# ZhaozhiQIAN/Hybrid-ODE-NeurIPS-2021

Hardware: AMD Instinct MI355X
Metric: patient-trajectories/sec (fwd+adjoint) at dim=12, T=100 (higher is better)
Workload: dtype f32; 1 GPU; dim12 synthetic, 10000 patients/GPU, T=100, dt=0.125, rk4(3/8), fused rhs+step kernel + discrete-adjoint kernel (split expert/learned wave pipelines); patients_total=10000, launch=hipGraph, lanes_per_patient=auto, theta_grad=True, parallelism=dp1, n_ranks=1, stage_tape=True

## Files before the change

hybrid-ode-neurips-2021_amd/csrc/hode_rk_split.hip:

```cpp
#include <hip/hip_runtime.h>
#include <stdlib.h>

#include "../../include/hode.h"
#include "hode_common.hpp"
#include "hode_host.hpp"
#include "hode_roche.hpp"

namespace hode {

#ifndef HODE_SPLIT_EXPERT_FIRST
#define HODE_SPLIT_EXPERT_FIRST 1
#endif
constexpr int kSplitPatients = 48;

struct SplitArgs {
  const float* __restrict__ t;
  const float* __restrict__ y0;
  const float* __restrict__ dosage;
  const float* __restrict__ dose_times;
  const float* __restrict__ theta;
  const float* __restrict__ w1;
  const float* __restrict__ b1;
  float* __restrict__ h;
  float* __restrict__ tape;
  unsigned long long* dbg;
  float* __restrict__ ltape;
  int* __restrict__ status;
  int B, T, K, perturb;
};

struct SpTimes {
  float t0, t1, dt, ts[4];
  HODE_DEV SpTimes(const float* __restrict__ t, int n, int perturb, int method) {
    t0 = t[n];
    t1 = t[n + 1];
    dt = t1 - t0;
    ts[0] = perturb ? nextafter_up(t0) : t0;
    ts[3] = perturb ? nextafter_down(t1) : t1;
    if (method == HODE_METHOD_RK4_38) {
      ts[1] = add_rn(t0, mul_rn(dt, (float)(1.0 / 3.0)));
      ts[2] = add_rn(t0, mul_rn(dt, (float)(2.0 / 3.0)));
    } else {
      ts[1] = add_rn(t0, mul_rn(0.5f, dt));
      ts[2] = ts[1];
    }
  }
};

template <int METHOD>
HODE_DEV float sp_stage_time(float t0, float t1, int perturb, int q) {
  const float dt = t1 - t0;
  const float c = METHOD == HODE_METHOD_RK4_38 ? (q == 1 ? (float)(1.0 / 3.0) : (q == 2 ? (float)(2.0 / 3.0) : 0.f))
                                               : (q == 0 ? 0.f : 0.5f);
  float tq = add_rn(t0, mul_rn(dt, c));
  tq = q == 3 ? t1 : tq;
  if (perturb) {
    if (q == 0) tq = nextafter_up(t0);
    if (q == 3) tq = nextafter_down(t1);
  }
  return tq;
}

constexpr int kSplitMaxT = 8192;
HODE_DEV void sp_stage_grid(float* __restrict__ tg, const float* __restrict__ t, int T) {
// ... 297 lines not shown
      for (int s = 0; s < NS; ++s) e[s] = *reinterpret_cast<const float4*>(&ring[par][s][slot][0]);
      __builtin_amdgcn_sched_barrier(0);
      dose_step(par, t_c, t_d);
#if HODE_SPLIT_EXPERT_FIRST
      typename Ml::Part pe[4];
#pragma unroll
      for (int s = 0; s < NS; ++s) pe[s] = ml.rhs_expert(e[s]);
#endif
#pragma unroll
      for (int s = 0; s < 4; ++s) k[s] = vsplat<Own>(0.f);
#pragma unroll
      for (int s = 0; s < NS; ++s) {
        const Own Yo = sp_stage_state<METHOD>(s, yo, dt, k[0], k[1], k[2]);
#if HODE_SPLIT_EXPERT_FIRST
        k[s] = ml.rhs_rest(pe[s], Ml::stage(e[s], Yo));
#else
        k[s] = ml.rhs(Ml::stage(e[s], Yo));
#endif
      }
      yo = sp_advance<METHOD>(yo, dt, k[0], k[1], k[2], k[3]);
      Ml::store_own(a.h + (size_t)(n + 1) * row + (size_t)p * D, q, yo);
      if constexpr (TAPE && NLT > 0) Ml::template store_tape<NLT>(a.ltape + (size_t)n * lt_step + lt_lane, k + (NS - NLT));
      HODE_FSTAMP(it)
      __syncthreads();
    };
    for (int it = 1; it < a.T; it += 2) {
      m_iter(it, IC<0>{});
      if (it + 1 < a.T) m_iter(it + 1, IC<1>{});
    }
    if (a.status) {
      if (!vfinite(yo) && live) atomicOr(a.status, HODE_STATUS_NONFINITE);
    }
  }
}

struct SplitBwdArgs {
  const float* __restrict__ t;
  const float* __restrict__ dosage;
  const float* __restrict__ dose_times;
  const float* __restrict__ theta;
  const float* __restrict__ w1;
  const float* __restrict__ b1;
  const float* __restrict__ h;
  const float* __restrict__ grad_h;
  float* __restrict__ grad_y0;
  float* __restrict__ part_ml;
  float* __restrict__ part_th;
  const float* __restrict__ tape;
  const float* __restrict__ ltape;
  int B, T, K, perturb;
  unsigned long long* dbg;
};

template <int METHOD, class V, class F>
HODE_DEV void sp_adjoint_step(V& lam, float dt, F&& vjp) {
  constexpr float c13 = (float)(1.0 / 3.0);
  if constexpr (METHOD == HODE_METHOD_EULER) {
    lam += vjp(0, dt * lam);
  } else if constexpr (METHOD == HODE_METHOD_MIDPOINT) {
    const V a1 = vjp(1, dt * lam);
    lam += a1;
    lam += vjp(0, (0.5f * dt) * a1);
  } else {
    const float w1 = dt * 0.125f, w3 = dt * 0.375f;
    const V a3 = vjp(3, w1 * lam);
    V da = dt * a3;
    V g1 = vfma(w1, lam, da);
    V g2 = vfma(w3, lam, -da);
    const V g = vfma(w3, lam, da);
    lam += a3;
    const V a2 = vjp(2, g);
    da = dt * a2;
    g2 += da;
    g1 = vfma(-c13, da, g1);
    lam += a2;
    const V a1 = vjp(1, g2);
    g1 = vfma(c13, dt * a1, g1);
    lam += a1;
    lam += vjp(0, g1);
  }
}

struct F4 {
  f2 a, b;
  HODE_DEV F4& operator+=(const F4& o) { a += o.a; b += o.b; return *this; }
  HODE_DEV F4 operator-() const { return F4{-a, -b}; }
};
HODE_DEV F4 operator*(float s, const F4& v) { return F4{s * v.a, s * v.b}; }
HODE_DEV F4 vfma(float s, const F4& x, const F4& y) { return F4{vfma(s, x.a, y.a), vfma(s, x.b, y.b)}; }

template <int D, bool CW>
struct SplitBwdShared {
  static constexpr int RD = CW ? 3 : 2;
  static constexpr int M = D - 4;
  float yring[RD][4][kSplitPatients][4];
  float cring[RD][4][kSplitPatients + 1][4];
  float dring[RD][kSplitPatients][8];
  float gring[RD][4][kSplitPatients + 1][4];
  float tdring[RD][kSplitPatients][8];
  float uring[CW ? RD : 1][4][CW ? kSplitPatients : 1][CW ? M : 1];
  float red[4][4][M * D + M];
};

template <int D, int METHOD, bool ABLATE, bool HILL2, bool NEED_TH, bool K1, bool TAPE>
HODE_DEV void split_bwd_body(const SplitBwdArgs& a, SplitBwdShared<D, TAPE>& sh) {
  constexpr int NS = sp_stages<METHOD>();
  typedef MlRows<D> Ml;
  typedef typename Ml::Own Own;
  constexpr int M = Ml::M, MR = Ml::MR, DP = Ml::DP, MP = Ml::MP;
  constexpr bool THW = TAPE && NEED_TH;
  constexpr bool CW = TAPE;
  constexpr int RD = SplitBwdShared<D, TAPE>::RD;
  constexpr int EL = CW ? 2 : 1;
  constexpr int CWAVE = THW ? 5 : 4;
  auto& yring = sh.yring; auto& cring = sh.cring; auto& dring = sh.dring; auto& gring = sh.gring;
  auto& tdring = sh.tdring; auto& uring = sh.uring; auto& red = sh.red;
  extern __shared__ float tg[];
  const int tid = threadIdx.x;
  const int wave = tid >> 6, lane = tid & 63;
  const int b0 = blockIdx.x * kSplitPatients;
  const RocheTheta th = load_theta(a.theta, ABLATE);
  const size_t row = (size_t)a.B * D;
  const int T = a.T;
  const int NIT = T + EL - 1;
  sp_stage_grid(tg, a.t, a.T);
#ifdef HODE_SPLIT_STAMPS
#define HODE_SSTAMP(k) if (a.dbg && blockIdx.x == 0 && lane == 0) a.dbg[(size_t)wave * (a.T + 2) + (k)] = __builtin_amdgcn_s_memtime();
#define HODE_PSTAMP(k, ph) { __builtin_amdgcn_sched_barrier(0); if (a.dbg && blockIdx.x == 0 && wave == 3 && lane == 0) a.dbg[(size_t)6 * (a.T + 2) + 64 + (size_t)(k) * 8 + (ph)] = __builtin_amdgcn_s_memtime(); __builtin_amdgcn_sched_barrier(0); }
  if (a.dbg && blockIdx.x < 8 && lane == 0) a.dbg[(size_t)6 * (a.T + 2) + blockIdx.x * 8 + wave] = __builtin_amdgcn_s_getreg(63492);
#else
#define HODE_SSTAMP(k)
#define HODE_PSTAMP(k, ph)
#endif
  auto run = [&](auto&& iter) {
    for (int k = 0; k < NIT; k += RD) {
      iter(k, IC<0>{});
      if (k + 1 < NIT) iter(k + 1, IC<1>{});
      if constexpr (RD == 3) {
        if (k + 2 < NIT) iter(k + 2, IC<2>{});
      }
    }
  };

  if (wave == 0) {
    const int slot = lane < kSplitPatients ? lane : 0;
    const bool mine = lane < kSplitPatients;
    const bool live = mine && b0 + slot < a.B;
    const int p = min(b0 + slot, a.B - 1);
    const float lv = live ? 1.0f : 0.0f;
    DoseSched<K1> ds;
    ds.dosage = a.dosage[p];
    ds.K = a.K;
    ds.taus = a.dose_times + (size_t)p * a.K;
    ds.tau0 = K1 ? ds.taus[0] : 0.f;
    const float ln_ec50 = log_f32(th.ec50);
    const int cslot = mine ? lane : kSplitPatients;
    if (lane < 16 * RD) (&cring[lane >> 4][(lane >> 2) & 3][kSplitPatients][0])[lane & 3] = 0.f;
    const unsigned lane_h = (unsigned)p * D, lane_t = (unsigned)p * 4;
    MlSlice<4, 1> none;
    MlColSlice<4, 1> nonec;
    GradAcc<4, 1> acc;
    acc.zero();
    float own1[1] = {0.f};

    float tp[4][4];
    auto fetch = [&](int m) {
      const float4 v = *reinterpret_cast<const float4*>(a.h + (size_t)m * row + lane_h);
      tp[0][0] = v.x; tp[0][1] = v.y; tp[0][2] = v.z; tp[0][3] = v.w;
      if constexpr (TAPE) {
        const float* __restrict__ tape_m = a.tape + (size_t)m * (NS - 1) * a.B * 4;
#pragma unroll
        for (int s = 1; s < NS; ++s) {
          const float4 u = *reinterpret_cast<const float4*>(tape_m + ((unsigned)(s - 1) * (unsigned)a.B * 4u + lane_t));
          tp[s][0] = u.x; tp[s][1] = u.y; tp[s][2] = u.z; tp[s][3] = u.w;
        }
      }
    };
    auto publish = [&](int m, int par) {
      if constexpr (TAPE) {
        if (mine) {
#pragma unroll
          for (int s = 0; s < NS; ++s)
            *reinterpret_cast<float4*>(&yring[par][s][slot][0]) = make_float4(tp[s][0], tp[s][1], tp[s][2], tp[s][3]);
        }
      } else {
        const SpTimes st(a.t, m, a.perturb, METHOD);
        const f2 ya = pair2(tp[0][0], tp[0][1]), yb = pair2(tp[0][2], tp[0][3]);
        f2 ka[4], kb[4];
#pragma unroll
        for (int s = 0; s < 4; ++s) ka[s] = kb[s] = splat2(0.f);
#pragma unroll
        for (int s = 0; s < NS; ++s) {
          const f2 Ya = sp_stage_state<METHOD>(s, ya, st.dt, ka[0], ka[1], ka[2]);
          const f2 Yb = sp_stage_state<METHOD>(s, yb, st.dt, kb[0], kb[1], kb[2]);
          const DoseVal dv = ds.at(st.ts[s], th.kel);
          if (mine) {
            *reinterpret_cast<float4*>(&yring[par][s][slot][0]) = make_float4(Ya.x, Ya.y, Yb.x, Yb.y);
            dring[par][slot][s] = dv.v;
            dring[par][slot][4 + s] = dv.dk;
          }
          if (s + 1 < NS) {
            const float Y[4] = {Ya.x, Ya.y, Yb.x, Yb.y};
            float k[4];
            roche_rhs<4, 1, ABLATE, HILL2>(th, none, dv.v, Y, k, own1);
            ka[s] = pair2(k[0], k[1]);
            kb[s] = pair2(k[2], k[3]);
          }
        }
      }
    };

    F4 lam;
    {
      const float4 g4 = *reinterpret_cast<const float4*>(a.grad_h + (size_t)(T - 1) * row + (size_t)p * D);
      lam.a = lv * pair2(g4.x, g4.y);
      lam.b = lv * pair2(g4.z, g4.w);
    }
    if (T >= 2) {
      fetch(T - 2);
      publish(T - 2, 0);
    }
    __syncthreads();
    auto e_iter = [&](int k, auto SI) {
      constexpr int S = decltype(SI)::value;
      constexpr int par = (S + 1) % RD;
      if (T - 3 - k >= 0) fetch(T - 3 - k);
      if (k >= EL && k <= T + EL - 2) {
        const int m = T - k + EL - 2;
        const float dt = tg[m + 1] - tg[m];
        float Y[4][4];
        F4 cs[4];
        DoseVal dv[4];
        {
          const float4 d0 = *reinterpret_cast<const float4*>(&dring[par][slot][0]);
          const float4 d1 = *reinterpret_cast<const float4*>(&dring[par][slot][4]);
          dv[0].v = d0.x; dv[1].v = d0.y; dv[2].v = d0.z; dv[3].v = d0.w;
          dv[0].dk = d1.x; dv[1].dk = d1.y; dv[2].dk = d1.z; dv[3].dk = d1.w;
          if constexpr (THW) {
            *reinterpret_cast<float4*>(&tdring[S][slot][0]) = d0;
            *reinterpret_cast<float4*>(&tdring[S][slot][4]) = d1;
          }
        }
#pragma unroll
        for (int s = 0; s < NS; ++s) {
          const float4 yv = *reinterpret_cast<const float4*>(&yring[par][s][slot][0]);
          const float4 cv = *reinterpret_cast<const float4*>(&cring[par][s][cslot][0]);
          Y[s][0] = yv.x; Y[s][1] = yv.y; Y[s][2] = yv.z; Y[s][3] = yv.w;
          cs[s].a = pair2(cv.x, cv.y);
          cs[s].b = pair2(cv.z, cv.w);
        }
        sp_adjoint_step<METHOD>(lam, dt, [&](int s, const F4& gs) {
          const float g[4] = {gs.a.x, gs.a.y, gs.b.x, gs.b.y};
          float av[4];
          if constexpr (THW) {
            if (mine) *reinterpret_cast<float4*>(&gring[S][s][slot][0]) = make_float4(g[0], g[1], g[2], g[3]);
          }
          roche_vjp<4, 1, ABLATE, HILL2, NEED_TH && !THW>(th, none, nonec, ln_ec50, dv[s], Y[s], own1, g, 0, av, acc);
          F4 r = cs[s];
          r.a += pair2(av[0], av[1]);
          r.b += pair2(av[2], av[3]);
          return r;
        });
        const float4 g4 = *reinterpret_cast<const float4*>(a.grad_h + (size_t)m * row + lane_h);
        lam.a = vfma(lv, pair2(g4.x, g4.y), lam.a);
        lam.b = vfma(lv, pair2(g4.z, g4.w), lam.b);
      }
      if (T - 3 - k >= 0) publish(T - 3 - k, par);
      HODE_SSTAMP(k)
      __syncthreads();
    };
    run(e_iter);
    if (live) *reinterpret_cast<float4*>(a.grad_y0 + (size_t)p * D) = make_float4(lam.a.x, lam.a.y, lam.b.x, lam.b.y);
    if constexpr (!THW) {
#pragma unroll
      for (int i = 0; i < kNTheta; ++i) {
        const float v = row_sum(NEED_TH ? acc.dth[i] : 0.f);
        if ((lane & 15) == 0) red[0][lane >> 4][i] = v;
      }
      __builtin_amdgcn_fence(__ATOMIC_SEQ_CST, "wavefront");
      if (lane < kNTheta)
        a.part_th[(size_t)blockIdx.x * kNTheta + lane] = (red[0][0][lane] + red[0][1][lane]) + (red[0][2][lane] + red[0][3][lane]);
    }
  } else if (THW && wave == 4) {
    const int slot = lane < kSplitPatients ? lane : 0;
    const bool mine = lane < kSplitPatients;
    const int p = min(b0 + slot, a.B - 1);
    const int gslot = mine ? lane : kSplitPatients;
    const float ln_ec50 = log_f32(th.ec50);
    if (lane < 16 * RD) (&gring[lane >> 4][(lane >> 2) & 3][kSplitPatients][0])[lane & 3] = 0.f;
    const unsigned lane_h = (unsigned)p * D, lane_t = (unsigned)p * 4;
    float dth[kNTheta];
#pragma unroll
    for (int i = 0; i < kNTheta; ++i) dth[i] = 0.f;
    float tp[4][4];
    auto fetch = [&](int m) {
      const float4 v = *reinterpret_cast<const float4*>(a.h + (size_t)m * row + lane_h);
      tp[0][0] = v.x; tp[0][1] = v.y; tp[0][2] = v.z; tp[0][3] = v.w;
      const float* __restrict__ tape_m = a.tape + (size_t)m * (NS - 1) * a.B * 4;
#pragma unroll
      for (int s = 1; s < NS; ++s) {
        const float4 u = *reinterpret_cast<const float4*>(tape_m + ((unsigned)(s - 1) * (unsigned)a.B * 4u + lane_t));
        tp[s][0] = u.x; tp[s][1] = u.y; tp[s][2] = u.z; tp[s][3] = u.w;
      }
    };
    auto theta_step = [&](int gpar) {
      const float4 d0 = *reinterpret_cast<const float4*>(&tdring[gpar][slot][0]);
      const float4 d1 = *reinterpret_cast<const float4*>(&tdring[gpar][slot][4]);
      const float dvv[4] = {d0.x, d0.y, d0.z, d0.w}, dvk[4] = {d1.x, d1.y, d1.z, d1.w};
#pragma unroll
      for (int si = 0; si < NS; ++si) {
        const int s = NS - 1 - si;
        const float4 gv = *reinterpret_cast<const float4*>(&gring[gpar][s][gslot][0]);
        DoseVal dv;
        dv.v = dvv[s]; dv.dk = dvk[s];
        const float g[4] = {gv.x, gv.y, gv.z, gv.w};
        roche_theta_grad<ABLATE, HILL2>(th, ln_ec50, dv, tp[s], g, dth);
      }
    };
    __syncthreads();
    auto t_iter = [&](int k, auto SI) {
      constexpr int S = decltype(SI)::value;
      constexpr int gpar = (S + RD - 1) % RD;
      if (k >= EL + 1) theta_step(gpar);
      if (k >= EL && T - k + EL - 2 >= 0) fetch(T - k + EL - 2);
      HODE_SSTAMP(k)
      __syncthreads();
    };
    run(t_iter);
    if (T >= 2) theta_step((NIT - 1) % RD);
#pragma unroll
    for (int i = 0; i < kNTheta; ++i) {
      const float v = row_sum(dth[i]);
      if ((lane & 15) == 0) red[0][lane >> 4][i] = v;
    }
    __builtin_amdgcn_fence(__ATOMIC_SEQ_CST, "wavefront");
    if (lane < kNTheta)
      a.part_th[(size_t)blockIdx.x * kNTheta + lane] = (red[0][0][lane] + red[0][1][lane]) + (red[0][2][lane] + red[0][3][lane]);
  } else if (CW && wave == CWAVE) {
    const int slot = lane < kSplitPatients ? lane : 0;
    const bool mine = lane < kSplitPatients;
    float wq[M][4];
#pragma unroll
    for (int j = 0; j < M; ++j)
#pragma unroll
      for (int q = 0; q < 4; ++q) wq[j][q] = a.w1[j * D + q];
    __syncthreads();
    auto c_iter = [&](int k, auto SI) {
      constexpr int S = decltype(SI)::value;
      constexpr int cpar = (S + RD - 1) % RD;
      if (k >= 1 && k - 1 <= T - 2) {
        float u[NS][M];
#pragma unroll
        for (int s = 0; s < NS; ++s) {
#pragma unroll
          for (int j4 = 0; j4 < M; j4 += 4) {
            const float4 v = *reinterpret_cast<const float4*>(&uring[cpar][s][slot][j4]);
            u[s][j4] = v.x; u[s][j4 + 1] = v.y; u[s][j4 + 2] = v.z; u[s][j4 + 3] = v.w;
          }
        }
        __builtin_amdgcn_sched_barrier(0);
#pragma unroll
        for (int s = 0; s < NS; ++s) {
          float c[4];
#pragma unroll
          for (int q = 0; q < 4; ++q) {
            if constexpr (MR == 2) {
              float cq = 0.f;
#pragma unroll
              for (int j = 0; j < M; ++j) cq = __builtin_fmaf(wq[j][q], u[s][j], cq);
              c[q] = cq;
            } else {
              float cx = 0.f, cy = 0.f;
#pragma unroll
              for (int jp = 0; jp < MP; ++jp) {
                cx = __builtin_fmaf(wq[2 * jp][q], u[s][2 * jp], cx);
                cy = __builtin_fmaf(wq[2 * jp + 1][q], u[s][2 * jp + 1], cy);
              }
              c[q] = cx + cy;
            }
          }
          if (mine) *reinterpret_cast<float4*>(&cring[cpar][s][slot][0]) = make_float4(c[0], c[1], c[2], c[3]);
        }
      }
      HODE_SSTAMP(k)
      __syncthreads();
    };
    run(c_iter);
  } else {
    const int q = lane & 3;
    const int slot = (wave - 1) * 16 + (lane >> 2);
    const bool live = b0 + slot < a.B;
    const int p = min(b0 + slot, a.B - 1);
    const float lv = live ? 1.0f : 0.0f;
    Ml ml;
    ml.load(a.w1, a.b1, q);
    typename Ml::Elem wc[Ml::NU];
    f2 wtp[Ml::NU];
    if constexpr (MR == 2) {
#pragma unroll
      for (int j = 0; j < M; ++j) {
        wc[j] = a.w1[j * D + q];
        wtp[j] = pair2(a.w1[j * D + 4 + 2 * q], a.w1[j * D + 4 + 2 * q + 1]);
      }
    } else {
#pragma unroll
      for (int jp = 0; jp < MP; ++jp) {
        wc[jp] = pair2(a.w1[(2 * jp) * D + q], a.w1[(2 * jp + 1) * D + q]);
        wtp[jp] = pair2(a.w1[(2 * jp) * D + 4 + q], a.w1[(2 * jp + 1) * D + 4 + q]);
      }
    }
    f2 dw[Ml::NW];
    Own db = vsplat<Own>(0.f);
#pragma unroll
    for (int i = 0; i < Ml::NW; ++i) dw[i] = splat2(0.f);
    DoseSched<K1> ds;
    ds.dosage = a.dosage[p];
    ds.K = a.K;
    ds.taus = a.dose_times + (size_t)p * a.K;
    ds.tau0 = K1 ? ds.taus[0] : 0.f;
    Own lam = lv * Ml::load_own(a.grad_h + (size_t)(T - 1) * row + (size_t)p * D, q);
    Own yo_nx, gh_nx;
    constexpr int NLT = TAPE ? sp_ltape_stages<METHOD>() : 0;
    const size_t lt_step = (size_t)a.B * 4 * NLT * MR;
    const unsigned lt_lane = ((unsigned)p * 4 + q) * NLT * MR;
    Own lt_nx[NLT > 0 ? NLT : 1], lt_n2[NLT > 0 ? NLT : 1];
    {
      const int m0 = T >= 2 ? T - 2 : 0;
      const int m1 = m0 >= 1 ? m0 - 1 : 0;
      yo_nx = Ml::load_own(a.h + (size_t)m0 * row + (size_t)p * D, q);
      gh_nx = Ml::load_own(a.grad_h + (size_t)m0 * row + (size_t)p * D, q);
      if constexpr (NLT > 0) {
        Ml::template load_tape<NLT>(a.ltape + (size_t)m0 * lt_step + lt_lane, lt_nx);
        Ml::template load_tape<NLT>(a.ltape + (size_t)m1 * lt_step + lt_lane, lt_n2);
      }
    }
    __syncthreads();
    auto m_iter = [&](int k, auto SI) {
      constexpr int par = decltype(SI)::value;
      if (k <= T - 2) {
        HODE_PSTAMP(k, 0)
        const int m = T - 2 - k;
        const float t0 = tg[m], t1 = tg[m + 1];
        const float dt = t1 - t0;
        const Own yo = yo_nx, gh = gh_nx;
        Own lt[NLT > 0 ? NLT : 1];
#pragma unroll
        for (int i = 0; i < NLT; ++i) { lt[i] = lt_nx[i]; lt_nx[i] = lt_n2[i]; }
        {
          const int mn = m >= 1 ? m - 1 : 0;
          yo_nx = Ml::load_own(a.h + (size_t)mn * row + (size_t)p * D, q);
          gh_nx = Ml::load_own(a.grad_h + (size_t)mn * row + (size_t)p * D, q);
          if constexpr (NLT > 0) Ml::template load_tape<NLT>(a.ltape + (size_t)(m >= 2 ? m - 2 : 0) * lt_step + lt_lane, lt_n2);
        }
        typename Ml::Stage Y[4];
        Own so[4];
        float4 e[4];
#pragma unroll
        for (int s = 0; s < NS; ++s) e[s] = *reinterpret_cast<const float4*>(&yring[par][s][slot][0]);
        __builtin_amdgcn_sched_barrier(0);
        HODE_PSTAMP(k, 1)
        if constexpr (TAPE) {
          const DoseVal dq = ds.at(sp_stage_time<METHOD>(t0, t1, a.perturb, q), th.kel);
          dring[par][slot][q] = dq.v;
          if constexpr (NEED_TH) dring[par][slot][4 + q] = dq.dk;
        }
#if HODE_SPLIT_EXPERT_FIRST
        typename Ml::Part pe[4];
#pragma unroll
        for (int s = 0; s < NS - NLT; ++s) pe[s] = ml.rhs_expert(e[s]);
#endif
#pragma unroll
        for (int s = 0; s < 4; ++s) so[s] = vsplat<Own>(0.f);
#pragma unroll
        for (int s = 0; s < NS; ++s) {
          const Own Yo = sp_stage_state<METHOD>(s, yo, dt, so[0], so[1], so[2]);
          Y[s] = Ml::stage(e[s], Yo);
          if (s >= NS - NLT) so[s] = lt[s - (NS - NLT) < 0 ? 0 : s - (NS - NLT)];
#if HODE_SPLIT_EXPERT_FIRST
          else so[s] = ml.rhs_rest(pe[s], Y[s]);
#else
          else so[s] = ml.rhs(Y[s]);
#endif
        }
        HODE_PSTAMP(k, 2)
        sp_adjoint_step<METHOD>(lam, dt, [&](int s, Own gs) {
          HODE_PSTAMP(k, 6 - s)
          const Own u = gs * vfma(-so[s], so[s], vsplat<Own>(1.0f));
          db += u;
          Ml::outer_acc(dw, u, Y[s]);
          if constexpr (CW) {
            if constexpr (MR == 2) *reinterpret_cast<float2*>(&uring[par][s][slot][2 * q]) = make_float2(u.x, u.y);
            else uring[par][s][slot][q] = u;
          }
          typename Ml::Gath uf;
          Ml::gather(u, uf.v);
          if constexpr (MR == 2) {
            float cq = 0.f;
            f2 av = splat2(0.f), av1 = splat2(0.f);
#pragma unroll
            for (int j = 0; j < M; j += 2) {
              if constexpr (!CW) cq = __builtin_fmaf(wc[j], uf.v[j], cq);
              av = vfma(wtp[j], uf.v[j], av);
              if constexpr (!CW) cq = __builtin_fmaf(wc[j + 1], uf.v[j + 1], cq);
              av1 = vfma(wtp[j + 1], uf.v[j + 1], av1);
            }
            if constexpr (!CW) cring[par][s][slot][q] = cq;
            return av + av1;
          } else {
            f2 c2 = splat2(0.f), a2 = splat2(0.f);
#pragma unroll
            for (int jp = 0; jp < MP; ++jp) {
              if constexpr (!CW) c2 = vfma(wc[jp], uf.v[jp], c2);
              a2 = vfma(wtp[jp], uf.v[jp], a2);
            }
            if constexpr (!CW) cring[par][s][slot][q] = hsum(c2);
            return hsum(a2);
          }
        });
        lam = vfma(lv, gh, lam);
        HODE_PSTAMP(k, 7)
      }
      HODE_SSTAMP(k)
      __syncthreads();
    };
    run(m_iter);
    if (live) Ml::store_own(a.grad_y0 + (size_t)p * D, q, lam);
    float* out = a.part_ml + ((size_t)blockIdx.x * 3 + (wave - 1)) * (M * D + M);
    const bool writer = (lane & 15) < 4;
    float* mine = &red[wave][lane >> 4][0];
#pragma unroll
    for (int r = 0; r < MR; ++r) {
#pragma unroll
      for (int i = 0; i < D; ++i) {
        const float v = row_sum_stride4(Ml::dw_at(dw, r, i));
        if (writer) mine[(q * MR + r) * D + i] = v;
      }
      float dbr;
      if constexpr (MR == 2) dbr = r == 0 ? db.x : db.y;
      else dbr = db;
      const float vb = row_sum_stride4(dbr);
      if (writer) mine[M * D + q * MR + r] = vb;
    }
    __builtin_amdgcn_fence(__ATOMIC_SEQ_CST, "wavefront");
    for (int c = lane; c < M * D + M; c += 64)
      out[c] = (red[wave][0][c] + red[wave][1][c]) + (red[wave][2][c] + red[wave][3][c]);
  }
}

__global__ __launch_bounds__(64) void split_fold_kernel(const float* __restrict__ part_ml, const float* __restrict__ part_th,
                                                        int nblk, int P_ml, int n_w, float* __restrict__ gw,
                                                        float* __restrict__ gb, float* __restrict__ gth, int need_th,
                                                        int overwrite) {
  const int j = blockIdx.x;
  const int lane = threadIdx.x;
  const bool ml = j < P_ml;
  const float* src = ml ? part_ml + j : part_th + (j - P_ml);
  const int rows = ml ? 3 * nblk : nblk;
  const int stride = ml ? P_ml : kNTheta;
  float s = 0.f;
  for (int base = 0; base < rows; base += 64 * 8) {
    float v[8];
#pragma unroll
    for (int q = 0; q < 8; ++q) {
      const int w = base + lane + 64 * q;
      v[q] = w < rows ? src[(size_t)w * stride] : 0.f;
    }
#pragma unroll
    for (int q = 0; q < 8; ++q) s += v[q];
  }
  s = wave_sum(s);
  if (lane != 0) return;
  float* dst = nullptr;
  if (ml) dst = j < n_w ? (gw ? gw + j : nullptr) : (gb ? gb + (j - n_w) : nullptr);
  else if (gth) dst = gth + (j - P_ml);
  if (!dst) return;
  if (!ml && !need_th) s = 0.f;
  *dst = overwrite ? s : *dst + s;
}

#ifndef HODE_SPLIT_WPE_FWD
#define HODE_SPLIT_WPE_FWD 2
#endif
#ifndef HODE_SPLIT_WPE_BWD
#define HODE_SPLIT_WPE_BWD 2
#endif
#ifndef HODE_SPLIT_WPE_BWD_MIN
#define HODE_SPLIT_WPE_BWD_MIN 1
#endif

template <int D, int METHOD, bool ABLATE, bool NEED_TH, bool TAPE>
__global__ __launch_bounds__(384) __attribute__((amdgpu_waves_per_eu(HODE_SPLIT_WPE_BWD_MIN, HODE_SPLIT_WPE_BWD))) void split_bwd_kernel(SplitBwdArgs a) {
  __shared__ __attribute__((aligned(16))) SplitBwdShared<D, TAPE> sh;
  const bool hill2 = ABLATE || (a.theta[0] == 2.0f && a.theta[1] == 2.0f);
  if (hill2 && a.K == 1) split_bwd_body<D, METHOD, ABLATE, true, NEED_TH, true, TAPE>(a, sh);
  else if (hill2) split_bwd_body<D, METHOD, ABLATE, true, NEED_TH, false, TAPE>(a, sh);
  else split_bwd_body<D, METHOD, ABLATE, false, NEED_TH, false, TAPE>(a, sh);
}

template <int D, int METHOD, bool ABLATE, bool TAPE>
__global__ __launch_bounds__(256) __attribute__((amdgpu_waves_per_eu(1, HODE_SPLIT_WPE_FWD))) void split_fwd_kernel(SplitArgs a) {
  const bool hill2 = ABLATE || (a.theta[0] == 2.0f && a.theta[1] == 2.0f);
  if (hill2 && a.K == 1) split_fwd_body<D, METHOD, ABLATE, true, true, TAPE>(a);
  else if (hill2) split_fwd_body<D, METHOD, ABLATE, true, false, TAPE>(a);
  else split_fwd_body<D, METHOD, ABLATE, false, false, TAPE>(a);
}

}

namespace {

template <int D, bool ABLATE>
int split_method(const hode_solve_desc* d, const hode::SplitArgs& a, hipStream_t s) {
  const dim3 grid((d->batch + hode::kSplitPatients - 1) / hode::kSplitPatients), block(256);
  const size_t lds = (size_t)(d->n_times + 3) * sizeof(float);
#define HODE_SPLIT_FWD(M)                                                                                 \
  if (a.tape) hipLaunchKernelGGL((hode::split_fwd_kernel<D, M, ABLATE, true>), grid, block, lds, s, a);   \
  else hipLaunchKernelGGL((hode::split_fwd_kernel<D, M, ABLATE, false>), grid, block, lds, s, a);
  switch (d->method) {
    case HODE_METHOD_EULER: HODE_SPLIT_FWD(HODE_METHOD_EULER) break;
    case HODE_METHOD_MIDPOINT: HODE_SPLIT_FWD(HODE_METHOD_MIDPOINT) break;
    default: HODE_SPLIT_FWD(HODE_METHOD_RK4_38) break;
  }
  return hode::hip_fail(hipGetLastError(), "split kernel launch");
}

}

namespace {

template <int D, bool ABLATE>
int split_bwd_method(const hode_solve_desc* d, const hode::SplitBwdArgs& a, hipStream_t s) {
  const dim3 grid((d->batch + hode::kSplitPatients - 1) / hode::kSplitPatients), block(256);
  const size_t lds = (size_t)(d->n_times + 3) * sizeof(float);
#define HODE_SPLIT_BWD(M)                                                                                        \
  if (d->need_theta_grad) {                                                                                      \
    if (a.tape) hipLaunchKernelGGL((hode::split_bwd_kernel<D, M, ABLATE, true, true>), grid, dim3(384), lds, s, a); \
    else hipLaunchKernelGGL((hode::split_bwd_kernel<D, M, ABLATE, true, false>), grid, block, lds, s, a);          \
  } else {                                                                                                       \
    if (a.tape) hipLaunchKernelGGL((hode::split_bwd_kernel<D, M, ABLATE, false, true>), grid, dim3(320), lds, s, a); \
    else hipLaunchKernelGGL((hode::split_bwd_kernel<D, M, ABLATE, false, false>), grid, block, lds, s, a);         \
  }
  switch (d->method) {
    case HODE_METHOD_EULER: HODE_SPLIT_BWD(HODE_METHOD_EULER) break;
    case HODE_METHOD_MIDPOINT: HODE_SPLIT_BWD(HODE_METHOD_MIDPOINT) break;
    default: HODE_SPLIT_BWD(HODE_METHOD_RK4_38) break;
  }
  return hode::hip_fail(hipGetLastError(), "split bwd kernel launch");
}

}

namespace hode {

bool split_supported(const hode_solve_desc* d) { return (d->latent_dim == 8 || d->latent_dim == 12) && d->n_times <= kSplitMaxT; }

static size_t al256s(size_t x) { return (x + 255) / 256 * 256; }

static int n_stages(int method) { return method == HODE_METHOD_EULER ? 1 : (method == HODE_METHOD_MIDPOINT ? 2 : 4); }

static size_t split_partials_bytes(const hode_solve_desc* d) {
  const size_t nblk = (d->batch + kSplitPatients - 1) / kSplitPatients;
  const size_t M = d->latent_dim - 4;
  return al256s(nblk * 3 * (M * d->latent_dim + M) * sizeof(float)) + al256s(nblk * kNTheta * sizeof(float));
}
static size_t split_etape_bytes(const hode_solve_desc* d) {
  if (!(d->flags & HODE_FLAG_TAPE) || d->n_times < 2) return 0;
  return al256s((size_t)(d->n_times - 1) * (n_stages(d->method) - 1) * d->batch * 4 * sizeof(float));
}
static size_t split_ltape_bytes(const hode_solve_desc* d) {
  if (!(d->flags & HODE_FLAG_TAPE) || d->n_times < 2 || n_stages(d->method) != 4 || kLearnedTapeStages == 0) return 0;
  return al256s((size_t)(d->n_times - 1) * d->batch * (d->latent_dim - 4) * kLearnedTapeStages * sizeof(float));
}
static size_t split_tape_bytes(const hode_solve_desc* d) { return split_etape_bytes(d) + split_ltape_bytes(d); }
size_t split_workspace_bytes(const hode_solve_desc* d) { return split_partials_bytes(d) + split_tape_bytes(d); }
static float* split_tape(const hode_solve_desc* d) {
  return split_etape_bytes(d) ? (float*)((char*)d->workspace + split_partials_bytes(d)) : nullptr;
}
static float* split_ltape(const hode_solve_desc* d) {
  return split_ltape_bytes(d) ? (float*)((char*)d->workspace + split_partials_bytes(d) + split_etape_bytes(d)) : nullptr;
}

int split_rk_bwd(const hode_solve_desc* d, hipStream_t s) {
  const int nblk = (d->batch + kSplitPatients - 1) / kSplitPatients;
  const int M = d->latent_dim - 4;
  const int Pml = M * d->latent_dim + M;
  char* ws = (char*)d->workspace;
  SplitBwdArgs a{};
  a.t = d->t; a.dosage = d->dosage; a.dose_times = d->dose_times; a.theta = d->theta; a.w1 = d->w1; a.b1 = d->b1;
  a.h = d->h; a.grad_h = d->grad_h; a.grad_y0 = d->grad_y0;
// ... 37 lines not shown
```

Measured before the change: 75.94 million trajectories/s.

## Offload learned-weight outer-product accumulation to helper waves in adjoint kernel

In the theta-grad tape configuration, the adjoint kernel grows from 6 to 8 waves. The dW outer-product accumulation and the c-vector computation move off the main learned-adjoint waves onto new helper waves, which read the learned-part stage states that the main waves now stage through a new LDS ring. The intent is to shorten the critical path of the serial adjoint waves by spreading that work across more waves. The cost is more LDS, more threads per block with waves_per_eu min 2 (tighter register budget), and an extra stage-state write per stage.

New measurement: 76.57 million trajectories/s (median of 6 runs). No clear change (+0.8%).

```diff
diff --git a/hybrid-ode-neurips-2021_amd/csrc/hode_rk_split.hip b/hybrid-ode-neurips-2021_amd/csrc/hode_rk_split.hip
--- a/hybrid-ode-neurips-2021_amd/csrc/hode_rk_split.hip
+++ b/hybrid-ode-neurips-2021_amd/csrc/hode_rk_split.hip
@@ -450,7 +450,7 @@
 HODE_DEV F4 operator*(float s, const F4& v) { return F4{s * v.a, s * v.b}; }
 HODE_DEV F4 vfma(float s, const F4& x, const F4& y) { return F4{vfma(s, x.a, y.a), vfma(s, x.b, y.b)}; }
 
-template <int D, bool CW>
+template <int D, bool CW, bool HW = false>
 struct SplitBwdShared {
   static constexpr int RD = CW ? 3 : 2;
   static constexpr int M = D - 4;
@@ -460,22 +460,25 @@
   float gring[RD][4][kSplitPatients + 1][4];
   float tdring[RD][kSplitPatients][8];
   float uring[CW ? RD : 1][4][CW ? kSplitPatients : 1][CW ? M : 1];
+  float ylring[HW ? RD : 1][4][HW ? kSplitPatients : 1][HW ? M : 1];
   float red[4][4][M * D + M];
 };
 
 template <int D, int METHOD, bool ABLATE, bool HILL2, bool NEED_TH, bool K1, bool TAPE>
-HODE_DEV void split_bwd_body(const SplitBwdArgs& a, SplitBwdShared<D, TAPE>& sh) {
+HODE_DEV void split_bwd_body(const SplitBwdArgs& a, SplitBwdShared<D, TAPE, TAPE && NEED_TH>& sh) {
   constexpr int NS = sp_stages<METHOD>();
   typedef MlRows<D> Ml;
   typedef typename Ml::Own Own;
   constexpr int M = Ml::M, MR = Ml::MR, DP = Ml::DP, MP = Ml::MP;
   constexpr bool THW = TAPE && NEED_TH;
   constexpr bool CW = TAPE;
-  constexpr int RD = SplitBwdShared<D, TAPE>::RD;
+  constexpr bool HW = THW;
+  constexpr int RD = SplitBwdShared<D, TAPE, HW>::RD;
   constexpr int EL = CW ? 2 : 1;
-  constexpr int CWAVE = THW ? 5 : 4;
+  constexpr int CWAVE = 4;
+  constexpr int HWAVE0 = 4;
   auto& yring = sh.yring; auto& cring = sh.cring; auto& dring = sh.dring; auto& gring = sh.gring;
-  auto& tdring = sh.tdring; auto& uring = sh.uring; auto& red = sh.red;
+  auto& tdring = sh.tdring; auto& uring = sh.uring; auto& ylring = sh.ylring; auto& red = sh.red;
   extern __shared__ float tg[];
   const int tid = threadIdx.x;
   const int wave = tid >> 6, lane = tid & 63;
@@ -487,8 +490,8 @@
   sp_stage_grid(tg, a.t, a.T);
 #ifdef HODE_SPLIT_STAMPS
 #define HODE_SSTAMP(k) if (a.dbg && blockIdx.x == 0 && lane == 0) a.dbg[(size_t)wave * (a.T + 2) + (k)] = __builtin_amdgcn_s_memtime();
-#define HODE_PSTAMP(k, ph) { __builtin_amdgcn_sched_barrier(0); if (a.dbg && blockIdx.x == 0 && wave == 3 && lane == 0) a.dbg[(size_t)6 * (a.T + 2) + 64 + (size_t)(k) * 8 + (ph)] = __builtin_amdgcn_s_memtime(); __builtin_amdgcn_sched_barrier(0); }
-  if (a.dbg && blockIdx.x < 8 && lane == 0) a.dbg[(size_t)6 * (a.T + 2) + blockIdx.x * 8 + wave] = __builtin_amdgcn_s_getreg(63492);
+#define HODE_PSTAMP(k, ph) { __builtin_amdgcn_sched_barrier(0); if (a.dbg && blockIdx.x == 0 && wave == 3 && lane == 0) a.dbg[(size_t)8 * (a.T + 2) + 64 + (size_t)(k) * 8 + (ph)] = __builtin_amdgcn_s_memtime(); __builtin_amdgcn_sched_barrier(0); }
+  if (a.dbg && blockIdx.x < 8 && lane == 0) a.dbg[(size_t)8 * (a.T + 2) + blockIdx.x * 8 + wave] = __builtin_amdgcn_s_getreg(63492);
 #else
 #define HODE_SSTAMP(k)
 #define HODE_PSTAMP(k, ph)
@@ -501,6 +504,30 @@
         if (k + 2 < NIT) iter(k + 2, IC<2>{});
       }
     }
+  };
+  auto ml_epilogue = [&](const f2 (&dw)[Ml::NW], Own db, int lw, int q, auto PART) {
+    constexpr int part = decltype(PART)::value;
+    float* out = a.part_ml + ((size_t)blockIdx.x * 3 + (lw - 1)) * (M * D + M);
+    const bool writer = (lane & 15) < 4;
+    float* mine = &red[lw][lane >> 4][0];
+#pragma unroll
+    for (int r = 0; r < MR; ++r) {
+#pragma unroll
+      for (int i = 0; i < (part == 2 ? 0 : D); ++i) {
+        const float v = row_sum_stride4(Ml::dw_at(dw, r, i));
+        if (writer) mine[(q * MR + r) * D + i] = v;
+      }
+      if constexpr (part != 1) {
+        float dbr;
+        if constexpr (MR == 2) dbr = r == 0 ? db.x : db.y;
+        else dbr = db;
+        const float vb = row_sum_stride4(dbr);
+        if (writer) mine[M * D + q * MR + r] = vb;
+      }
+    }
+    __builtin_amdgcn_fence(__ATOMIC_SEQ_CST, "wavefront");
+    for (int c = (part == 2 ? M * D : 0) + lane; c < (part == 1 ? M * D : M * D + M); c += 64)
+      out[c] = (red[lw][0][c] + red[lw][1][c]) + (red[lw][2][c] + red[lw][3][c]);
   };
 
   if (wave == 0) {
@@ -697,7 +724,80 @@
     __builtin_amdgcn_fence(__ATOMIC_SEQ_CST, "wavefront");
     if (lane < kNTheta)
       a.part_th[(size_t)blockIdx.x * kNTheta + lane] = (red[0][0][lane] + red[0][1][lane]) + (red[0][2][lane] + red[0][3][lane]);
-  } else if (CW && wave == CWAVE) {
+  } else if (HW && wave > HWAVE0) {
+    if constexpr (HW) {
+    const int lw = wave - HWAVE0;
+    const int q = lane & 3;
+    const int slot = (lw - 1) * 16 + (lane >> 2);
+    float wq[M];
+#pragma unroll
+    for (int j = 0; j < M; ++j) wq[j] = a.w1[j * D + q];
+    f2 dw[Ml::NW];
+#pragma unroll
+    for (int i = 0; i < Ml::NW; ++i) dw[i] = splat2(0.f);
+    __syncthreads();
+    auto h_iter = [&](int k, auto SI) {
+      constexpr int S = decltype(SI)::value;
+      constexpr int cpar = (S + RD - 1) % RD;
+      if (k >= 1 && k - 1 <= T - 2) {
+        float4 e[NS];
+        float yl[NS][M], u[NS][M];
+        Own uo[NS];
+#pragma unroll
+        for (int s = 0; s < NS; ++s) {
+          e[s] = *reinterpret_cast<const float4*>(&yring[cpar][s][slot][0]);
+#pragma unroll
+          for (int j4 = 0; j4 < M; j4 += 4) {
+            const float4 v = *reinterpret_cast<const float4*>(&uring[cpar][s][slot][j4]);
+            u[s][j4] = v.x; u[s][j4 + 1] = v.y; u[s][j4 + 2] = v.z; u[s][j4 + 3] = v.w;
+            const float4 y = *reinterpret_cast<const float4*>(&ylring[cpar][s][slot][j4]);
+            yl[s][j4] = y.x; yl[s][j4 + 1] = y.y; yl[s][j4 + 2] = y.z; yl[s][j4 + 3] = y.w;
+          }
+          if constexpr (MR == 2) {
+            const float2 v = *reinterpret_cast<const float2*>(&uring[cpar][s][slot][2 * q]);
+            uo[s] = pair2(v.x, v.y);
+          } else uo[s] = uring[cpar][s][slot][q];
+        }
+        __builtin_amdgcn_sched_barrier(0);
+#pragma unroll
+        for (int si = 0; si < NS; ++si) {
+          const int s = NS - 1 - si;
+          typename Ml::Stage Y;
+          if constexpr (MR == 2) {
+            Y.v[0] = e[s].x; Y.v[1] = e[s].y; Y.v[2] = e[s].z; Y.v[3] = e[s].w;
+#pragma unroll
+            for (int j = 0; j < M; ++j) Y.v[4 + j] = yl[s][j];
+          } else {
+            Y.v[0] = pair2(e[s].x, e[s].y);
+            Y.v[1] = pair2(e[s].z, e[s].w);
+            Y.v[2] = pair2(yl[s][0], yl[s][1]);
+            Y.v[3] = pair2(yl[s][2], yl[s][3]);
+          }
+          Ml::outer_acc(dw, uo[s], Y);
+          float cq;
+          if constexpr (MR == 2) {
+            cq = 0.f;
+#pragma unroll
+            for (int j = 0; j < M; ++j) cq = __builtin_fmaf(wq[j], u[s][j], cq);
+          } else {
+            float cx = 0.f, cy = 0.f;
+#pragma unroll
+            for (int jp = 0; jp < MP; ++jp) {
+              cx = __builtin_fmaf(wq[2 * jp], u[s][2 * jp], cx);
+              cy = __builtin_fmaf(wq[2 * jp + 1], u[s][2 * jp + 1], cy);
+            }
+            cq = cx + cy;
+          }
+          cring[cpar][s][slot][q] = cq;
+        }
+      }
+      HODE_SSTAMP(k)
+      __syncthreads();
+    };
+    run(h_iter);
+    ml_epilogue(dw, vsplat<Own>(0.f), lw, q, IC<1>{});
+    }
+  } else if (CW && !HW && wave == CWAVE) {
     const int slot = lane < kSplitPatients ? lane : 0;
     const bool mine = lane < kSplitPatients;
     float wq[M][4];
@@ -817,7 +917,7 @@
         Own so[4];
         float4 e[4];
 #pragma unroll
-        for (int s = 0; s < NS; ++s) e[s] = *reinterpret_cast<const float4*>(&yring[par][s][slot][0]);
+        for (int s = 0; s < (HW ? NS - NLT : NS); ++s) e[s] = *reinterpret_cast<const float4*>(&yring[par][s][slot][0]);
         __builtin_amdgcn_sched_barrier(0);
         HODE_PSTAMP(k, 1)
         if constexpr (TAPE) {
@@ -835,7 +935,13 @@
 #pragma unroll
         for (int s = 0; s < NS; ++s) {
           const Own Yo = sp_stage_state<METHOD>(s, yo, dt, so[0], so[1], so[2]);
-          Y[s] = Ml::stage(e[s], Yo);
+          if constexpr (HW) {
+            if constexpr (MR == 2) *reinterpret_cast<float2*>(&ylring[par][s][slot][2 * q]) = make_float2(Yo.x, Yo.y);
+            else ylring[par][s][slot][q] = Yo;
+            if (s < NS - NLT) Y[s] = Ml::stage(e[s], Yo);
+          } else {
+            Y[s] = Ml::stage(e[s], Yo);
+          }
           if (s >= NS - NLT) so[s] = lt[s - (NS - NLT) < 0 ? 0 : s - (NS - NLT)];
 #if HODE_SPLIT_EXPERT_FIRST
           else so[s] = ml.rhs_rest(pe[s], Y[s]);
@@ -848,7 +954,7 @@
           HODE_PSTAMP(k, 6 - s)
           const Own u = gs * vfma(-so[s], so[s], vsplat<Own>(1.0f));
           db += u;
-          Ml::outer_acc(dw, u, Y[s]);
+          if constexpr (!HW) Ml::outer_acc(dw, u, Y[s]);
           if constexpr (CW) {
             if constexpr (MR == 2) *reinterpret_cast<float2*>(&uring[par][s][slot][2 * q]) = make_float2(u.x, u.y);
             else uring[par][s][slot][q] = u;
@@ -886,25 +992,8 @@
     };
     run(m_iter);
     if (live) Ml::store_own(a.grad_y0 + (size_t)p * D, q, lam);
-    float* out = a.part_ml + ((size_t)blockIdx.x * 3 + (wave - 1)) * (M * D + M);
-    const bool writer = (lane & 15) < 4;
-    float* mine = &red[wave][lane >> 4][0];
-#pragma unroll
-    for (int r = 0; r < MR; ++r) {
-#pragma unroll
-      for (int i = 0; i < D; ++i) {
-        const float v = row_sum_stride4(Ml::dw_at(dw, r, i));
-        if (writer) mine[(q * MR + r) * D + i] = v;
-      }
-      float dbr;
-      if constexpr (MR == 2) dbr = r == 0 ? db.x : db.y;
-      else dbr = db;
-      const float vb = row_sum_stride4(dbr);
-      if (writer) mine[M * D + q * MR + r] = vb;
-    }
-    __builtin_amdgcn_fence(__ATOMIC_SEQ_CST, "wavefront");
-    for (int c = lane; c < M * D + M; c += 64)
-      out[c] = (red[wave][0][c] + red[wave][1][c]) + (red[wave][2][c] + red[wave][3][c]);
+    if constexpr (HW) ml_epilogue(dw, db, wave, q, IC<2>{});
+    else ml_epilogue(dw, db, wave, q, IC<0>{});
   }
 }
 
@@ -950,8 +1039,8 @@
 #endif
 
 template <int D, int METHOD, bool ABLATE, bool NEED_TH, bool TAPE>
-__global__ __launch_bounds__(384) __attribute__((amdgpu_waves_per_eu(HODE_SPLIT_WPE_BWD_MIN, HODE_SPLIT_WPE_BWD))) void split_bwd_kernel(SplitBwdArgs a) {
-  __shared__ __attribute__((aligned(16))) SplitBwdShared<D, TAPE> sh;
+__global__ __launch_bounds__(NEED_TH && TAPE ? 512 : 384) __attribute__((amdgpu_waves_per_eu(NEED_TH && TAPE ? 2 : HODE_SPLIT_WPE_BWD_MIN, HODE_SPLIT_WPE_BWD))) void split_bwd_kernel(SplitBwdArgs a) {
+  __shared__ __attribute__((aligned(16))) SplitBwdShared<D, TAPE, TAPE && NEED_TH> sh;
   const bool hill2 = ABLATE || (a.theta[0] == 2.0f && a.theta[1] == 2.0f);
   if (hill2 && a.K == 1) split_bwd_body<D, METHOD, ABLATE, true, NEED_TH, true, TAPE>(a, sh);
   else if (hill2) split_bwd_body<D, METHOD, ABLATE, true, NEED_TH, false, TAPE>(a, sh);
@@ -995,7 +1084,7 @@
   const size_t lds = (size_t)(d->n_times + 3) * sizeof(float);
 #define HODE_SPLIT_BWD(M)                                                                                        \
   if (d->need_theta_grad) {                                                                                      \
-    if (a.tape) hipLaunchKernelGGL((hode::split_bwd_kernel<D, M, ABLATE, true, true>), grid, dim3(384), lds, s, a); \
+    if (a.tape) hipLaunchKernelGGL((hode::split_bwd_kernel<D, M, ABLATE, true, true>), grid, dim3(512), lds, s, a); \
     else hipLaunchKernelGGL((hode::split_bwd_kernel<D, M, ABLATE, true, false>), grid, block, lds, s, a);          \
   } else {                                                                                                       \
     if (a.tape) hipLaunchKernelGGL((hode::split_bwd_kernel<D, M, ABLATE, false, true>), grid, dim3(320), lds, s, a); \
```

## Restructure learned-wave adjoint VJP with rotated W layout and DPP reduction

Applied to the files above, without the earlier changes.

Replaces the gather-then-dot VJP for the learned block (MR==2) with a rotated per-lane W_LL layout, so each lane multiplies its own u and the lanes reduce with two DPP swizzles instead of gathering all M entries. For RK4 3/8 it also reorders the adjoint step so the first stage's dt/8 weight is folded into the tanh-derivative factor. It moves the grad_h join to before the last VJP, which shortens the serial dependency chain on lam. Shared ring arrays are flattened through index helpers. The risk is extra registers for the rotated weights and changed floating-point rounding order.

After: 75.98 million trajectories/s before, 76.75 million trajectories/s after (median of 6 runs). 1.01x the previous value.

```diff
diff --git a/hybrid-ode-neurips-2021_amd/csrc/hode_rk_split.hip b/hybrid-ode-neurips-2021_amd/csrc/hode_rk_split.hip
--- a/hybrid-ode-neurips-2021_amd/csrc/hode_rk_split.hip
+++ b/hybrid-ode-neurips-2021_amd/csrc/hode_rk_split.hip
@@ -10,6 +10,12 @@
 
 #ifndef HODE_SPLIT_EXPERT_FIRST
 #define HODE_SPLIT_EXPERT_FIRST 1
+#endif
+#ifndef HODE_SPLIT_VJP_SCATTER
+#define HODE_SPLIT_VJP_SCATTER 1
+#endif
+#ifndef HODE_SPLIT_ADJ_ONE_LINK
+#define HODE_SPLIT_ADJ_ONE_LINK 1
 #endif
 constexpr int kSplitPatients = 48;
 
@@ -413,15 +419,35 @@
   unsigned long long* dbg;
 };
 
-template <int METHOD, class V, class F>
-HODE_DEV void sp_adjoint_step(V& lam, float dt, F&& vjp) {
+template <int METHOD, bool ONE_LINK, class V, class F, class J>
+HODE_DEV void sp_adjoint_step(V& lam, float dt, F&& vjp, J&& join) {
   constexpr float c13 = (float)(1.0 / 3.0);
   if constexpr (METHOD == HODE_METHOD_EULER) {
     lam += vjp(0, dt * lam);
+    lam = join(lam);
   } else if constexpr (METHOD == HODE_METHOD_MIDPOINT) {
     const V a1 = vjp(1, dt * lam);
     lam += a1;
     lam += vjp(0, (0.5f * dt) * a1);
+    lam = join(lam);
+  } else if constexpr (ONE_LINK) {
+    const float w1 = dt * 0.125f, w3 = dt * 0.375f, cdt = c13 * dt;
+    const V wl1 = w1 * lam, wl3 = w3 * lam;
+    const V a3 = vjp(3, lam);
+    const V g = vfma(dt, a3, wl3);
+    const V t2 = vfma(-dt, a3, wl3);
+    V t1 = vfma(dt, a3, wl1);
+    V s = lam;
+    s += a3;
+    const V a2 = vjp(2, g);
+    const V g2 = vfma(dt, a2, t2);
+    t1 = vfma(-cdt, a2, t1);
+    s += a2;
+    const V a1 = vjp(1, g2);
+    const V g1 = vfma(cdt, a1, t1);
+    s += a1;
+    lam = join(s);
+    lam += vjp(0, g1);
   } else {
     const float w1 = dt * 0.125f, w3 = dt * 0.375f;
     const V a3 = vjp(3, w1 * lam);
@@ -439,6 +465,7 @@
     g1 = vfma(c13, dt * a1, g1);
     lam += a1;
     lam += vjp(0, g1);
+    lam = join(lam);
   }
 }
 
@@ -450,17 +477,59 @@
 HODE_DEV F4 operator*(float s, const F4& v) { return F4{s * v.a, s * v.b}; }
 HODE_DEV F4 vfma(float s, const F4& x, const F4& y) { return F4{vfma(s, x.a, y.a), vfma(s, x.b, y.b)}; }
 
+constexpr int wll_rot_col(int q, int r, int c) { return 2 * (r ^ q) + c; }
+constexpr bool wll_rot_covers_once() {
+  int seen[64] = {};
+  for (int q = 0; q < 4; ++q)
+    for (int r = 0; r < 4; ++r)
+      for (int h = 0; h < 2; ++h)
+        for (int c = 0; c < 2; ++c) ++seen[(2 * q + h) * 8 + wll_rot_col(q, r, c)];
+  for (int i = 0; i < 64; ++i)
+    if (seen[i] != 1) return false;
+  return true;
+}
+static_assert(wll_rot_covers_once(), "the rotated W_LL layout must hold every entry exactly once");
+
+struct WllRot {
+  f2 w[4][2];
+  HODE_DEV void load(const float* __restrict__ W, int q) {
+#pragma unroll
+    for (int r = 0; r < 4; ++r)
+#pragma unroll
+      for (int h = 0; h < 2; ++h) {
+        const float* __restrict__ src = W + (2 * q + h) * 12 + 4 + wll_rot_col(q, r, 0);
+        w[r][h] = pair2(src[0], src[1]);
+      }
+  }
+  HODE_DEV f2 vjp(f2 u) const {
+    f2 P[4];
+#pragma unroll
+    for (int r = 0; r < 4; ++r) P[r] = w[r][0] * splat2(u.x);
+    P[3] = vfma(w[3][1], u.y, P[3]);
+    P[2] = vfma(w[2][1], u.y, P[2]);
+    P[1] = vfma(w[1][1], u.y, P[1]);
+    P[0] = vfma(w[0][1], u.y, P[0]);
+    const float s1x = P[1].x + dpp_f32<0x4E>(P[3].x);
+    const float s1y = P[1].y + dpp_f32<0x4E>(P[3].y);
+    const float s0x = P[0].x + dpp_f32<0x4E>(P[2].x);
+    const float s0y = P[0].y + dpp_f32<0x4E>(P[2].y);
+    return pair2(s0x + dpp_f32<0xB1>(s1x), s0y + dpp_f32<0xB1>(s1y));
+  }
+};
+
 template <int D, bool CW>
 struct SplitBwdShared {
   static constexpr int RD = CW ? 3 : 2;
   static constexpr int M = D - 4;
   float yring[RD][4][kSplitPatients][4];
   float cring[RD][4][kSplitPatients + 1][4];
-  float dring[RD][kSplitPatients][8];
+  float dring[RD][kSplitPatients * 8];
   float gring[RD][4][kSplitPatients + 1][4];
-  float tdring[RD][kSplitPatients][8];
-  float uring[CW ? RD : 1][4][CW ? kSplitPatients : 1][CW ? M : 1];
+  float tdring[RD][kSplitPatients * 8];
+  float uring[CW ? RD : 1][4][CW ? kSplitPatients * M : 1];
   float red[4][4][M * D + M];
+  static HODE_DEV int dose_ix(int slot, int j) { return slot * 8 + j; }
+  static HODE_DEV int u_ix(int slot, int j) { return slot * M + j; }
 };
 
 template <int D, int METHOD, bool ABLATE, bool HILL2, bool NEED_TH, bool K1, bool TAPE>
@@ -471,7 +540,8 @@
   constexpr int M = Ml::M, MR = Ml::MR, DP = Ml::DP, MP = Ml::MP;
   constexpr bool THW = TAPE && NEED_TH;
   constexpr bool CW = TAPE;
-  constexpr int RD = SplitBwdShared<D, TAPE>::RD;
+  typedef SplitBwdShared<D, TAPE> Sh;
+  constexpr int RD = Sh::RD;
   constexpr int EL = CW ? 2 : 1;
   constexpr int CWAVE = THW ? 5 : 4;
   auto& yring = sh.yring; auto& cring = sh.cring; auto& dring = sh.dring; auto& gring = sh.gring;
@@ -557,8 +627,8 @@
           const DoseVal dv = ds.at(st.ts[s], th.kel);
           if (mine) {
             *reinterpret_cast<float4*>(&yring[par][s][slot][0]) = make_float4(Ya.x, Ya.y, Yb.x, Yb.y);
-            dring[par][slot][s] = dv.v;
-            dring[par][slot][4 + s] = dv.dk;
+            dring[par][Sh::dose_ix(slot, s)] = dv.v;
+            dring[par][Sh::dose_ix(slot, 4 + s)] = dv.dk;
           }
           if (s + 1 < NS) {
             const float Y[4] = {Ya.x, Ya.y, Yb.x, Yb.y};
@@ -593,13 +663,13 @@
         F4 cs[4];
         DoseVal dv[4];
         {
-          const float4 d0 = *reinterpret_cast<const float4*>(&dring[par][slot][0]);
-          const float4 d1 = *reinterpret_cast<const float4*>(&dring[par][slot][4]);
+          const float4 d0 = *reinterpret_cast<const float4*>(&dring[par][Sh::dose_ix(slot, 0)]);
+          const float4 d1 = *reinterpret_cast<const float4*>(&dring[par][Sh::dose_ix(slot, 4)]);
           dv[0].v = d0.x; dv[1].v = d0.y; dv[2].v = d0.z; dv[3].v = d0.w;
           dv[0].dk = d1.x; dv[1].dk = d1.y; dv[2].dk = d1.z; dv[3].dk = d1.w;
           if constexpr (THW) {
-            *reinterpret_cast<float4*>(&tdring[S][slot][0]) = d0;
-            *reinterpret_cast<float4*>(&tdring[S][slot][4]) = d1;
+            *reinterpret_cast<float4*>(&tdring[S][Sh::dose_ix(slot, 0)]) = d0;
+            *reinterpret_cast<float4*>(&tdring[S][Sh::dose_ix(slot, 4)]) = d1;
           }
         }
 #pragma unroll
@@ -610,7 +680,7 @@
           cs[s].a = pair2(cv.x, cv.y);
           cs[s].b = pair2(cv.z, cv.w);
         }
-        sp_adjoint_step<METHOD>(lam, dt, [&](int s, const F4& gs) {
+        sp_adjoint_step<METHOD, false>(lam, dt, [&](int s, const F4& gs) {
           const float g[4] = {gs.a.x, gs.a.y, gs.b.x, gs.b.y};
           float av[4];
           if constexpr (THW) {
@@ -621,10 +691,10 @@
           r.a += pair2(av[0], av[1]);
           r.b += pair2(av[2], av[3]);
           return r;
+        }, [&](const F4& x) {
+          const float4 g4 = *reinterpret_cast<const float4*>(a.grad_h + (size_t)m * row + lane_h);
+          return F4{vfma(lv, pair2(g4.x, g4.y), x.a), vfma(lv, pair2(g4.z, g4.w), x.b)};
         });
-        const float4 g4 = *reinterpret_cast<const float4*>(a.grad_h + (size_t)m * row + lane_h);
-        lam.a = vfma(lv, pair2(g4.x, g4.y), lam.a);
-        lam.b = vfma(lv, pair2(g4.z, g4.w), lam.b);
       }
       if (T - 3 - k >= 0) publish(T - 3 - k, par);
       HODE_SSTAMP(k)
@@ -665,8 +735,8 @@
       }
     };
     auto theta_step = [&](int gpar) {
-      const float4 d0 = *reinterpret_cast<const float4*>(&tdring[gpar][slot][0]);
-      const float4 d1 = *reinterpret_cast<const float4*>(&tdring[gpar][slot][4]);
+      const float4 d0 = *reinterpret_cast<const float4*>(&tdring[gpar][Sh::dose_ix(slot, 0)]);
+      const float4 d1 = *reinterpret_cast<const float4*>(&tdring[gpar][Sh::dose_ix(slot, 4)]);
       const float dvv[4] = {d0.x, d0.y, d0.z, d0.w}, dvk[4] = {d1.x, d1.y, d1.z, d1.w};
 #pragma unroll
       for (int si = 0; si < NS; ++si) {
@@ -715,7 +785,7 @@
         for (int s = 0; s < NS; ++s) {
 #pragma unroll
           for (int j4 = 0; j4 < M; j4 += 4) {
-            const float4 v = *reinterpret_cast<const float4*>(&uring[cpar][s][slot][j4]);
+            const float4 v = *reinterpret_cast<const float4*>(&uring[cpar][s][Sh::u_ix(slot, j4)]);
             u[s][j4] = v.x; u[s][j4 + 1] = v.y; u[s][j4 + 2] = v.z; u[s][j4 + 3] = v.w;
           }
         }
@@ -755,14 +825,18 @@
     const float lv = live ? 1.0f : 0.0f;
     Ml ml;
     ml.load(a.w1, a.b1, q);
+    constexpr bool SCATTER = MR == 2 && HODE_SPLIT_VJP_SCATTER;
+    constexpr bool FOLD_W1 = METHOD == HODE_METHOD_RK4_38 && HODE_SPLIT_ADJ_ONE_LINK;
     typename Ml::Elem wc[Ml::NU];
     f2 wtp[Ml::NU];
+    WllRot wrot;
     if constexpr (MR == 2) {
 #pragma unroll
       for (int j = 0; j < M; ++j) {
         wc[j] = a.w1[j * D + q];
         wtp[j] = pair2(a.w1[j * D + 4 + 2 * q], a.w1[j * D + 4 + 2 * q + 1]);
       }
+      if constexpr (SCATTER) wrot.load(a.w1, q);
     } else {
 #pragma unroll
       for (int jp = 0; jp < MP; ++jp) {
@@ -822,8 +896,8 @@
         HODE_PSTAMP(k, 1)
         if constexpr (TAPE) {
           const DoseVal dq = ds.at(sp_stage_time<METHOD>(t0, t1, a.perturb, q), th.kel);
-          dring[par][slot][q] = dq.v;
-          if constexpr (NEED_TH) dring[par][slot][4 + q] = dq.dk;
+          dring[par][Sh::dose_ix(slot, q)] = dq.v;
+          if constexpr (NEED_TH) dring[par][Sh::dose_ix(slot, 4 + q)] = dq.dk;
         }
 #if HODE_SPLIT_EXPERT_FIRST
         typename Ml::Part pe[4];
@@ -843,15 +917,28 @@
           else so[s] = ml.rhs(Y[s]);
 #endif
         }
+        Own ds2w = vsplat<Own>(0.f);
+        if constexpr (FOLD_W1) ds2w = (dt * 0.125f) * vfma(-so[NS - 1], so[NS - 1], vsplat<Own>(1.0f));
         HODE_PSTAMP(k, 2)
-        sp_adjoint_step<METHOD>(lam, dt, [&](int s, Own gs) {
+        sp_adjoint_step<METHOD, FOLD_W1>(lam, dt, [&](int s, Own gs) {
           HODE_PSTAMP(k, 6 - s)
-          const Own u = gs * vfma(-so[s], so[s], vsplat<Own>(1.0f));
+          const Own u = gs * (FOLD_W1 && s == NS - 1 ? ds2w : vfma(-so[s], so[s], vsplat<Own>(1.0f)));
           db += u;
           Ml::outer_acc(dw, u, Y[s]);
           if constexpr (CW) {
-            if constexpr (MR == 2) *reinterpret_cast<float2*>(&uring[par][s][slot][2 * q]) = make_float2(u.x, u.y);
-            else uring[par][s][slot][q] = u;
+            if constexpr (MR == 2) *reinterpret_cast<float2*>(&uring[par][s][Sh::u_ix(slot, 2 * q)]) = make_float2(u.x, u.y);
+            else uring[par][s][Sh::u_ix(slot, q)] = u;
+          }
+          if constexpr (SCATTER) {
+            if constexpr (!CW) {
+              typename Ml::Gath uf;
+              Ml::gather(u, uf.v);
+              float cq = 0.f;
+#pragma unroll
+              for (int j = 0; j < M; ++j) cq = __builtin_fmaf(wc[j], uf.v[j], cq);
+              cring[par][s][slot][q] = cq;
+            }
+            return wrot.vjp(u);
           }
           typename Ml::Gath uf;
           Ml::gather(u, uf.v);
@@ -877,8 +964,7 @@
             if constexpr (!CW) cring[par][s][slot][q] = hsum(c2);
             return hsum(a2);
           }
-        });
-        lam = vfma(lv, gh, lam);
+        }, [&](Own x) { return vfma(lv, gh, x); });
         HODE_PSTAMP(k, 7)
       }
       HODE_SSTAMP(k)
```
